# csiro-robotics/ohm

Hardware: AMD Instinct MI355X
Metric: rays/sec integrated (occupancy) (higher is better)
Workload: dtype f64

## Files before the change

### ohm_amd/csrc/batch_run.h

```cpp
#ifndef OHMHIP_BATCH_RUN_H
#define OHMHIP_BATCH_RUN_H

namespace
{
struct BatchRun
{
  ohmhip_map_t m;
  const double *d_rays;
  const float *d_intensities;
  const double *d_timestamps;
  uint32_t n_rays;
  unsigned ray_flags;
  hipStream_t s, f;
  const Event *tev;
  uint32_t ring;
  uint32_t next_info_index = 0;
  bool info_clean = false;
  uint32_t ray_blocks = 0, bin_rays_per_block = 0, bin_threads = 0, bin_blocks = 0, bin_tab_mask = 0;
  uint32_t batch_chunk_segments = 0;
  int mode = 0;
  bool stop_mode = false, occupancy_mode = false, ndt_mode = false, tsdf_mode = false;
  bool occ_inline = false;
  int ray_shift = 0;
  SecondaryLayers sec;
  int attempt = 0;
  uint32_t spec_seg_cap = 0, seg_cap = 0;
  bool speculated = false, bucket_hits = false;
  bool binned_early = false;
  BatchInfo info;
  unsigned long long *keys_a = nullptr, *keys_b = nullptr, *events = nullptr;
  const unsigned long long *sorted = nullptr;
  uint32_t event_capacity = 0, n_events = 0;
  float *direct_occ = nullptr;
  uint32_t direct_segments = 0;
  uint32_t sort_covers = 0;
  bool batch_end_marked = false;
  bool events_speculated = false;
  uint32_t spec_events = 0;

  uint32_t walkLdsHits() const { return uint32_t(m->walk_half ? WalkHalf::kLdsHits : WalkFull::kLdsHits); }

  void mark(int k) { m->tev_mask[ring] = uint8_t(m->tev_mask[ring] | (1u << k)); }

  int prepare()
  {
    m->tev_mask[ring] = 0;
    m->tev_pre_walk[ring] = 0;
    m->info_index = (m->info_index + 1u) % 3u;
    next_info_index = (m->info_index + 1u) % 3u;
    info_clean = m->info_clean;
    m->info_clean = false;
    m->parity ^= 1u;
    ray_blocks = (n_rays + 255) / 256;
    bin_rays_per_block = m->bin_rays_per_block;
    bin_threads = kBinThreads;
    while (bin_rays_per_block > 128 && n_rays / bin_rays_per_block < 2 * m->walk_workgroups)
    {
      bin_rays_per_block /= 2;
    }
    bin_threads = std::min<uint32_t>(bin_threads, bin_rays_per_block);
    bin_blocks = (n_rays + bin_rays_per_block - 1) / bin_rays_per_block;
    bin_tab_mask = std::min<uint32_t>(kLtabSize, std::max<uint32_t>(256u, 2u * bin_rays_per_block)) - 1u;
    const uint64_t expected_segments = uint64_t(double(n_rays) * m->segments_per_ray);
    batch_chunk_segments = m->chunk_segments;
    const uint32_t chunk_floor = (n_rays <= 16384u) ? std::min<uint32_t>(m->min_chunk_segments, 512u) : m->min_chunk_segments;
    while (batch_chunk_segments > chunk_floor &&
           expected_segments / batch_chunk_segments < 3ull * m->walkSlots())
    {
      batch_chunk_segments /= 2;
    }
    mode = m->config.mode;
    stop_mode = mode == OHMHIP_MODE_OCCUPANCY && (ray_flags & OHMHIP_RF_STOP_ON_FIRST_OCCUPIED) != 0;
    occupancy_mode = mode == OHMHIP_MODE_OCCUPANCY && !stop_mode;
    ndt_mode = mode == OHMHIP_MODE_NDT_OM || mode == OHMHIP_MODE_NDT_TM;
    tsdf_mode = mode == OHMHIP_MODE_TSDF;
    if (ndt_mode)
    {
      ray_flags &= (OHMHIP_RF_END_POINT_AS_FREE | OHMHIP_RF_EXCLUDE_ORIGIN | OHMHIP_RF_EXCLUDE_RAY);
    }
    if (tsdf_mode)
    {
      ray_flags = OHMHIP_RF_END_POINT_AS_FREE;
    }
    ray_shift = occupancy_mode ? 0 : kEvRayShift;
    sec.traversal = tsdf_mode ? nullptr : static_cast<float *>(m->pool.layers[OHMHIP_LID_TRAVERSAL].get());
    sec.touch_time = tsdf_mode ? nullptr : static_cast<uint32_t *>(m->pool.layers[OHMHIP_LID_TOUCH_TIME].get());
    sec.incident = tsdf_mode ? nullptr : static_cast<uint32_t *>(m->pool.layers[OHMHIP_LID_INCIDENT].get());
    sec.timestamps = d_timestamps;
    sec.time_base = m->first_ray_time;
    occ_inline = occupancy_mode && !m->pool.layers[OHMHIP_LID_MEAN] && !sec.traversal && !sec.touch_time && !sec.incident &&
                 !m->pool.layers[OHMHIP_LID_INTENSITY] && !m->pool.layers[OHMHIP_LID_HIT_MISS];

    for (int p = 0; p < 2; ++p)
    {
      OHMHIP_CHECK(m->walks_buf[p].ensure(sizeof(RayWalk) * size_t(n_rays), false, s));
      OHMHIP_CHECK(m->wg_regions[p].ensure(sizeof(WgRegion) * size_t(bin_blocks) * kLtabSize, false, s));
      OHMHIP_CHECK(m->wg_region_count[p].ensure(sizeof(uint32_t) * size_t(bin_blocks), false, s));
    }
    if (occupancy_mode)
    {
      OHMHIP_CHECK(m->hit_keys_a.ensure(sizeof(unsigned long long) * size_t(n_rays), false, s));
      OHMHIP_CHECK(m->hit_keys_b.ensure(sizeof(unsigned long long) * size_t(n_rays), false, s));
      OHMHIP_CHECK(m->interval_counts.ensure(sizeof(uint32_t) * size_t(n_rays), true, s));
      size_t sort_bytes = 0;
      OHMHIP_CHECK(rocprim::radix_sort_keys<SortConfig>(nullptr, sort_bytes, static_cast<unsigned long long *>(m->hit_keys_a.ptr),
                                            static_cast<unsigned long long *>(m->hit_keys_b.ptr), size_t(n_rays),
                                            kHitRayBits, sortEndBit(m), s));
      OHMHIP_CHECK(m->sort_temp.ensure(sort_bytes, false, s));
    }
    return OHMHIP_OK;
  }

  uint32_t *binMask() const { return occupancy_mode ? nullptr : m->pool.d_hit_mask.get(); }

  void launchBin(bool bucket, uint32_t seg_capacity, unsigned long long *hit_keys, hipStream_t stream)
  {
    const auto pow2 = [](int v) { return (v & (v - 1)) == 0; };
    const bool plain = m->mc.owner_world <= 1u && pow2(m->mc.dim[0]) && pow2(m->mc.dim[1]) && pow2(m->mc.dim[2]);
    const bool small = bin_tab_mask < kLtabSmall;
    const auto kernel = small ? (plain ? k_ray_bin<kLtabSmall, true> : k_ray_bin<kLtabSmall, false>) :
                                (plain ? k_ray_bin<kLtabSize, true> : k_ray_bin<kLtabSize, false>);
    hipExtLaunchKernelGGL(kernel, dim3(bin_blocks), dim3(bin_threads), 0, stream, nullptr, tev[1], 0, m->mc,
                          regionTable(m), batchScratch(m), static_cast<const RayWalk *>(batchWalks(m).ptr), n_rays,
                          static_cast<Segment *>(m->segments.ptr), seg_capacity, hit_keys, binMask(), ray_shift,
                          bucket ? 1 : 0, bin_rays_per_block, bin_tab_mask);
    mark(1);
    m->tev_pre_walk[ring] = 1;
    m->bin_done_event = tev[1];
  }

  uint32_t sortGrid(uint32_t per_cu) const
  {
    const uint32_t grid = per_cu * m->walk_workgroups;
    return m->sort_workgroups ? std::min(grid, m->sort_workgroups) : grid;
  }

  void launchRegionSort(uint32_t dense)
  {
    const unsigned long long *in = static_cast<const unsigned long long *>(m->hit_keys_a.ptr);
    unsigned long long *out = static_cast<unsigned long long *>(m->hit_keys_b.ptr);
    const bool need_dense = kSortSmallHits == 0 || dense > kSortSmallHits;
    if (need_dense)
    {
      hipExtLaunchKernelGGL((k_sort_region_hits<kSortRegionHits, kSortThreads>), dim3(sortGrid(2)),
                            dim3(kSortThreads), 0, s, nullptr, kSortSmallHits ? nullptr : tev[2].handle, 0, regionTable(m),
                            batchScratch(m), in, out, m->mc.region_voxels, kSortSmallHits, m->pool.d_hit_mask.get(),
                            m->d_order_counts.get());
    }
    if (kSortSmallHits)
    {
      hipExtLaunchKernelGGL((k_sort_region_hits<kSortSmallHits ? kSortSmallHits : 64u, kSortSmallThreads>),
                            dim3(sortGrid(8)), dim3(kSortSmallThreads), 0, s, nullptr, tev[2], 0,
                            regionTable(m), batchScratch(m), in, out, m->mc.region_voxels, 0u, m->pool.d_hit_mask.get(),
                            m->d_order_counts.get());
    }
    sort_covers = need_dense ? kSortRegionHits : kSortSmallHits;
    mark(2);
    m->tev_pre_walk[ring] = 2;
  }

  void launchDenseSort()
  {
    hipExtLaunchKernelGGL((k_sort_region_hits<kSortRegionHits, kSortThreads>), dim3(sortGrid(2)),
                          dim3(kSortThreads), 0, s, nullptr, tev[2], 0, regionTable(m), batchScratch(m),
                          static_cast<const unsigned long long *>(m->hit_keys_a.ptr),
                          static_cast<unsigned long long *>(m->hit_keys_b.ptr), m->mc.region_voxels, kSortSmallHits,
                          m->pool.d_hit_mask.get(), m->d_order_counts.get());
    sort_covers = kSortRegionHits;
  }

  int frontHalf()
  {
    if (m->batch_done_event[m->parity])
    {
      OHMHIP_CHECK(hipStreamWaitEvent(f, m->batch_done_event[m->parity], 0));
    }
    if (m->bin_done_event)
    {
      OHMHIP_CHECK(hipStreamWaitEvent(f, m->bin_done_event, 0));
    }
    if (attempt > 0 || !info_clean)
    {
      OHMHIP_CHECK(hipMemsetAsync(m->d_info + m->info_index, 0, sizeof(BatchInfo), f));
    }
    if (m->phase_timing)
    {
      OHMHIP_CHECK(hipEventRecord(tev[0], f));
      mark(0);
    }
    if (bin_tab_mask < kLtabSmall)
    {
      hipLaunchKernelGGL(k_ray_setup<kLtabSmall>, dim3(bin_blocks), dim3(bin_threads), 0, f, m->mc, regionTable(m),
                         batchScratch(m), d_rays, n_rays, ray_flags, static_cast<RayWalk *>(batchWalks(m).ptr),
                         bin_rays_per_block, bin_tab_mask);
    }
    else
    {
      hipLaunchKernelGGL(k_ray_setup<kLtabSize>, dim3(bin_blocks), dim3(bin_threads), 0, f, m->mc, regionTable(m),
                         batchScratch(m), d_rays, n_rays, ray_flags, static_cast<RayWalk *>(batchWalks(m).ptr),
                         bin_rays_per_block, bin_tab_mask);
    }
    hipExtLaunchKernelGGL(k_plan, dim3(1), dim3(1024), 0, f, nullptr, tev[5], 0, regionTable(m), batchScratch(m),
                          batchChunks(m), m->pool.chunk_capacity, batch_chunk_segments, m->h_info.dev,
                          m->d_info + next_info_index, batchEventCount(m), occ_inline ? walkLdsHits() : 0u);
    mark(5);
    m->info_clean = true;
    hipEvent_t plan_done = tev[5];
    if (m->spill_enabled)
    {
      OHMHIP_CHECK(queueUseStamps(m, f));
      OHMHIP_CHECK(hipEventRecord(m->ev[7], f));
      plan_done = m->ev[7];
    }
    OHMHIP_CHECK(hipStreamWaitEvent(s, plan_done, 0));
    spec_seg_cap = uint32_t(std::min<size_t>(m->segments.bytes / sizeof(Segment), 0xffffffffu));
    speculated = occupancy_mode && m->spec_bucket_ok && attempt == 0 && spec_seg_cap > 0;
    binned_early = speculated && m->early_bin && m->early_bin_event != nullptr;
    hipStream_t bin_stream = binned_early ? f : s;
    if (binned_early)
    {
      OHMHIP_CHECK(hipStreamWaitEvent(f, m->early_bin_event, 0));
    }
    if (m->phase_timing)
    {
      OHMHIP_CHECK(hipEventRecord(tev[6], bin_stream));
      mark(6);
    }
    if (speculated)
    {
      launchBin(true, spec_seg_cap, static_cast<unsigned long long *>(m->hit_keys_a.ptr), bin_stream);
      if (binned_early)
      {
        OHMHIP_CHECK(hipStreamWaitEvent(s, tev[1], 0));
        hipExtLaunchKernelGGL(k_stream_marker, dim3(1), dim3(64), 0, s, nullptr, tev[7], 0);
        m->bin_done_event = tev[7];
      }
      launchRegionSort(m->spec_max_region_hits);
    }
    OHMHIP_CHECK(hipEventSynchronize(plan_done));
    OHMHIP_CHECK(hipGetLastError());
    info = *m->h_info;
    return OHMHIP_OK;
  }

  bool exhausted() const
  {
    return (info.error & (kErrSlotsFull | kErrHashFull)) || info.n_slots > m->pool.slot_capacity ||
           info.n_chunks > m->pool.chunk_capacity;
  }

  int resolveExhaustion(bool &retry)
  {
    retry = false;
    OHMHIP_CHECK(hipStreamSynchronize(s));
    m->spec_bucket_ok = false;
    const int err = growPool(m, info.n_slots, m->pool.slot_capacity * 2u, m->slots_committed);
    if (err)
    {
      const int rollback_err = rollbackTable(m);
      if (rollback_err)
      {
        return rollback_err;
      }
      if (err == OHMHIP_ERR_CAPACITY && m->spill_enabled && !(info.error & kErrHashFull) &&
          info.n_slots > m->slots_committed)
      {
        const uint64_t allowed = poolBudget(m).regions;
        const uint64_t wanted = uint64_t(info.n_slots);
        m->batch_exceeds_limit = wanted > allowed && wanted - allowed > m->slots_committed;
        if (wanted > allowed && wanted - allowed <= m->slots_committed)
        {
          const int evict_err = evictColdRegions(m, uint32_t(wanted - allowed));
          if (evict_err == OHMHIP_OK)
          {
            retry = true;
            return OHMHIP_OK;
          }
        }
      }
      return err;
    }
    retry = true;
    return OHMHIP_OK;
  }

  int commitRegions()
  {
    m->cache_misses += info.n_slots - m->slots_committed;
    m->cache_hits += info.n_touched - std::min(info.n_touched, info.n_slots - m->slots_committed);
    if (!m->spilled.empty())
    {
      OHMHIP_CHECK(readmitSpilledSlots(m, m->slots_committed, info.n_slots));
    }
    m->slots_committed = info.n_slots;
    if (speculated && (info.n_segments > spec_seg_cap || info.max_region_hits > kSortRegionHits))
    {
      OHMHIP_CHECK(hipStreamSynchronize(s));
      if (info.n_touched)
      {
        hipLaunchKernelGGL(k_reset_cursors, dim3((info.n_touched + 255) / 256), dim3(256), 0, s, regionTable(m),
                           batchScratch(m));
      }
      speculated = false;
      binned_early = false;
    }
    return OHMHIP_OK;
  }

  int sizeBuffers()
  {
    OHMHIP_CHECK(m->segments.ensure(sizeof(Segment) * size_t(std::max<uint32_t>(info.n_segments, 1u)), false, s));
    seg_cap = uint32_t(std::min<size_t>(m->segments.bytes / sizeof(Segment), 0xffffffffu));

    uint64_t want_events =
      std::max<uint64_t>({ uint64_t(1) << 20, info.visits / 4, uint64_t(m->event_demand) * 5 / 4 });
    want_events = std::min<uint64_t>(want_events, 0xfffffff0ull - n_rays);
    if (occupancy_mode)
    {
      const uint64_t have = m->events.bytes / sizeof(unsigned long long);
      if (have >= std::max<uint64_t>(uint64_t(1) << 20, 16ull * n_rays))
      {
        want_events = std::max<uint64_t>(std::min(want_events, have), uint64_t(m->event_demand) * 5 / 4);
      }
    }
    if (m->event_limit)
    {
      want_events = std::min<uint64_t>(want_events, m->event_limit);
    }
    keys_a = keys_b = events = nullptr;
    event_capacity = 0;
    if (occupancy_mode)
    {
      OHMHIP_CHECK(m->events.ensure(sizeof(unsigned long long) * size_t(want_events), false, s));
      keys_a = static_cast<unsigned long long *>(m->hit_keys_a.ptr);
      keys_b = static_cast<unsigned long long *>(m->hit_keys_b.ptr);
      events = static_cast<unsigned long long *>(m->events.ptr);
      event_capacity = uint32_t(std::min<size_t>(m->events.bytes / sizeof(unsigned long long), 0xfffffff0u));
    }
    else
    {
      const size_t total = size_t(n_rays) + size_t(want_events);
      OHMHIP_CHECK(m->hit_keys_a.ensure(sizeof(unsigned long long) * total, false, s));
      OHMHIP_CHECK(m->hit_keys_b.ensure(sizeof(unsigned long long) * total, false, s));
      keys_a = static_cast<unsigned long long *>(m->hit_keys_a.ptr);
      keys_b = static_cast<unsigned long long *>(m->hit_keys_b.ptr);
      events = keys_a + n_rays;
      const size_t cap_a = m->hit_keys_a.bytes / sizeof(unsigned long long) - n_rays;
      const size_t cap_b = m->hit_keys_b.bytes / sizeof(unsigned long long) - n_rays;
      event_capacity = uint32_t(std::min<size_t>(std::min(cap_a, cap_b), 0xfffffff0u - n_rays));
      if (m->event_limit)
      {
        event_capacity = std::min(event_capacity, m->event_limit);
      }
    }
    return OHMHIP_OK;
  }

  int binAndOrder()
  {
    bucket_hits = occupancy_mode && info.max_region_hits <= kSortRegionHits;
    m->spec_bucket_ok = bucket_hits;
    m->spec_max_region_hits = info.max_region_hits;
    if (m->debug_flags & 4096u)
    {
      std::fprintf(stderr, "[ohmhip dbg] batch: %u rays, %u segments, %u chunks, %u regions touched, %u with samples, "
                   "densest %u samples; binned speculatively: %d\n", n_rays, info.n_segments, info.n_chunks,
                   info.n_touched, info.n_hit_regions, info.max_region_hits, int(speculated));
    }
    sorted = keys_b;
    if (speculated && info.max_region_hits > sort_covers)
    {
      launchDenseSort();
    }
    if (!speculated)
    {
      launchBin(bucket_hits, seg_cap, keys_a, s);
      if (tsdf_mode)
      {
        hipExtLaunchKernelGGL(k_tsdf_flag, dim3(ray_blocks), dim3(256), 0, s, nullptr, tev[2], 0, m->mc, regionTable(m),
                              static_cast<const RayWalk *>(batchWalks(m).ptr), d_rays, n_rays, m->pool.d_hit_mask.get());
        mark(2);
        m->tev_pre_walk[ring] = 2;
      }
      if (bucket_hits)
      {
        if (info.n_hit_regions)
        {
          launchRegionSort(info.max_region_hits);
        }
      }
      else if (occupancy_mode)
      {
        size_t temp_bytes = m->sort_temp.bytes;
        OHMHIP_CHECK(rocprim::radix_sort_keys<SortConfig>(m->sort_temp.ptr, temp_bytes, keys_a, keys_b, size_t(n_rays),
                                                          kHitRayBits, sortEndBit(info.n_slots), s));
        hipExtLaunchKernelGGL(k_hit_bounds, dim3(ray_blocks), dim3(256), 0, s, nullptr, tev[2], 0, sorted,
                              batchScratch(m), m->mc.region_voxels, m->pool.d_hit_mask.get());
        mark(2);
        m->tev_pre_walk[ring] = 2;
      }
    }
    return OHMHIP_OK;
  }

  int walk(int first_attempt = 0)
  {
    direct_occ = (occupancy_mode || mode == OHMHIP_MODE_NDT_OM) ? static_cast<float *>(m->pool.layers[OHMHIP_LID_OCCUPANCY].get()) :
                                                                  nullptr;
    direct_segments = (direct_occ || tsdf_mode) ? batch_chunk_segments : 0u;
    n_events = 0;
    if (info.n_chunks)
    {
      for (int walk_attempt = first_attempt; walk_attempt < 4; ++walk_attempt)
      {
        if (walk_attempt > 0)
        {
          OHMHIP_CHECK(hipMemsetAsync(batchEventCount(m), 0, 2 * sizeof(uint32_t), s));
        }
        WalkArgs wa;
        wa.mc = m->mc;
        wa.bs = batchScratch(m);
        wa.chunks = batchChunks(m);
        wa.segments = static_cast<const Segment *>(m->segments.ptr);
        wa.walks = static_cast<const RayWalk *>(batchWalks(m).ptr);
        wa.slot_keys = m->pool.d_slot_keys;
        wa.sorted_hits = sorted;
        wa.hit_mask = m->pool.d_hit_mask;
        wa.miss_counts = m->pool.d_miss_counts;
        wa.interval_counts = static_cast<uint32_t *>(m->interval_counts.ptr);
        wa.events = events;
        wa.event_capacity = event_capacity;
        wa.event_count = batchEventCount(m);
        wa.refill_min_idle = m->refill_min_idle;
        wa.dbg = m->debug_flags;
        wa.ray_shift = ray_shift;
        wa.defer_all = occupancy_mode ? 0 : 1;
        wa.occupancy = direct_occ;
        wa.tsdf = tsdf_mode ? static_cast<float *>(m->pool.layers[OHMHIP_LID_TSDF].get()) : nullptr;
        wa.ray_flags = ray_flags;
        const bool trace = (m->debug_flags & (16u | 64u | 128u)) != 0;
        wa.dbg_counters = trace ? m->d_dbg : nullptr;
        wa.chunk_cursor = batchEventCount(m) + 1;
        wa.n_chunks = info.n_chunks;
        wa.rewalk = (walk_attempt > 0 && (direct_occ || tsdf_mode)) ? 1 : 0;
        wa.flag_all =
          ((tsdf_mode && (m->mc.tsdf_dropoff > 0 || m->mc.tsdf_max_weight > kTsdfCountedWeightLimit)) || stop_mode) ? 1 : 0;
        wa.inline_hits = occ_inline ? 1 : 0;
        const bool traversal_pass = sec.traversal != nullptr && walk_attempt == 0;
        const bool special = (ray_flags & OHMHIP_RF_EXCLUDE_ORIGIN) != 0;
        const dim3 wgrid(std::min<uint32_t>(info.n_chunks, m->walkSlots()));
        const dim3 wblock(m->walk_half ? WalkHalf::kThreads : WalkFull::kThreads);
        const size_t wlds = walkLdsBytes(m->mc, m->chunk_segments, m->walk_half);
        hipEvent_t walk_stop = traversal_pass ? nullptr : tev[3].handle;
        if (m->walk_half)
        {
          if (special)
          {
            hipExtLaunchKernelGGL((k_region_walk<true, false, WalkHalf>), wgrid, wblock, wlds, s, nullptr, walk_stop, 0, wa);
          }
          else if (trace)
          {
            hipExtLaunchKernelGGL((k_region_walk<false, true, WalkHalf>), wgrid, wblock, wlds, s, nullptr, walk_stop, 0, wa);
          }
          else
          {
            hipExtLaunchKernelGGL((k_region_walk<false, false, WalkHalf>), wgrid, wblock, wlds, s, nullptr, walk_stop, 0, wa);
          }
        }
        else if (special)
        {
// ... 353 lines not shown
```

### ohm_amd/csrc/sample_sort_kernels.h

```cpp
#ifndef OHMHIP_SAMPLE_SORT_KERNELS_H
#define OHMHIP_SAMPLE_SORT_KERNELS_H

#include "batch_scratch.h"
#include "region_table.h"

namespace ohmhip
{
__global__ void __launch_bounds__(256)
  k_hit_bounds(const unsigned long long *__restrict__ sorted, BatchScratch bs, int region_voxels,
               uint32_t *__restrict__ hit_mask)
{
  const uint32_t n_hits = bs.info->n_hits;
  const uint32_t i = blockIdx.x * blockDim.x + threadIdx.x;
  if (i >= n_hits)
  {
    return;
  }
  const unsigned long long group = hitGroup(sorted[i]);
  if (i == 0 || hitGroup(sorted[i - 1]) != group)
  {
    const uint32_t slot = hitSlot(sorted[i]);
    const uint32_t vi = hitVoxel(sorted[i]);
    bs.voxel_first_hit[size_t(slot) * size_t(region_voxels) + vi] = i;
    atomicOr(&hit_mask[size_t(slot) * (uint32_t(region_voxels + 31) >> 5) + (vi >> 5)], 1u << (vi & 31));
  }
  const uint32_t slot = hitSlot(sorted[i]);
  if (i == 0 || hitSlot(sorted[i - 1]) != slot)
  {
    bs.hit_begin[slot] = i;
  }
  if (i + 1 == n_hits || hitSlot(sorted[i + 1]) != slot)
  {
    bs.hit_end[slot] = i + 1;
  }
}

__device__ inline uint32_t sortSlot(uint32_t i)
{
  return i + (i >> 5);
}

template <int R>
__device__ inline void bitonicFused(unsigned long long *l_keys, uint32_t g, uint32_t s_shift, uint32_t k)
{
  constexpr uint32_t kCount = 1u << R;
  const uint32_t low = g & ((1u << s_shift) - 1u);
  const uint32_t base = ((g >> s_shift) << (s_shift + R)) | low;
  const bool ascending = (base & k) == 0;
  unsigned long long v[kCount];
#pragma unroll
  for (uint32_t m = 0; m < kCount; ++m)
  {
    v[m] = l_keys[sortSlot(base | (m << s_shift))];
  }
#pragma unroll
  for (int t = 0; t < R; ++t)
  {
    const uint32_t d = 1u << (R - 1 - t);
#pragma unroll
    for (uint32_t m = 0; m < kCount; ++m)
    {
      if ((m & d) == 0)
      {
        const unsigned long long a = v[m];
        const unsigned long long c = v[m | d];
        const bool swap = (a > c) == ascending;
        v[m] = swap ? c : a;
        v[m | d] = swap ? a : c;
      }
    }
  }
#pragma unroll
  for (uint32_t m = 0; m < kCount; ++m)
  {
    l_keys[sortSlot(base | (m << s_shift))] = v[m];
  }
}

template <int kThreads>
__device__ inline void bitonicNetwork(unsigned long long *l_keys, uint32_t padded, uint32_t tid)
{
  for (uint32_t k = 2; k <= padded; k <<= 1)
  {
    uint32_t j = k >> 1;
    while (j > 0)
    {
      const uint32_t levels_left = uint32_t(32 - __clz(int(j)));
      const uint32_t r = min(3u, levels_left);
      const uint32_t s_shift = levels_left - r;
      const uint32_t group_count = padded >> r;
      for (uint32_t g = tid; g < group_count; g += kThreads)
      {
        if (r == 3)
        {
          bitonicFused<3>(l_keys, g, s_shift, k);
        }
        else if (r == 2)
        {
          bitonicFused<2>(l_keys, g, s_shift, k);
        }
        else
        {
          bitonicFused<1>(l_keys, g, s_shift, k);
        }
      }
      __syncthreads();
      j >>= r;
    }
  }
}

constexpr uint32_t kSortRegionHits = 8192;
constexpr int kSortThreads = 1024;
#ifndef OHMHIP_SORT_SMALL
#define OHMHIP_SORT_SMALL 2048
#endif
constexpr uint32_t kSortSmallHits = OHMHIP_SORT_SMALL;
constexpr int kSortSmallThreads = 256;

#ifndef OHMHIP_ORDER_SHIFT_SMALL
#define OHMHIP_ORDER_SHIFT_SMALL 5
#endif
#ifndef OHMHIP_ORDER_SHIFT_DENSE
#define OHMHIP_ORDER_SHIFT_DENSE 5
#endif
#ifndef OHMHIP_ORDER_RANK_LIMIT
#define OHMHIP_ORDER_RANK_LIMIT 32
#endif
constexpr uint32_t kOrderRankLimit = OHMHIP_ORDER_RANK_LIMIT;
static_assert(kSortRegionHits < 65536u, "bucket positions are 16-bit halves");
constexpr unsigned long long kBelowSlot = (1ull << kHitSlotShift) - 1ull;
static_assert(kSortRegionHits <= (1u << (64 - kHitSlotShift)), "a key's final position travels in its slot field");

template <uint32_t kCap, int kThreads>
__global__ void __launch_bounds__(kThreads, 8)
  k_sort_region_hits(RegionTable rt, BatchScratch bs, const unsigned long long *__restrict__ keys,
                     unsigned long long *__restrict__ sorted, int region_voxels, uint32_t min_hits,
                     uint32_t *__restrict__ hit_mask, unsigned long long *__restrict__ order_counts)
{
  constexpr uint32_t kPerLane = (kCap + uint32_t(kThreads) - 1u) / uint32_t(kThreads);
  constexpr uint32_t kWaves = uint32_t(kThreads) / 64u;
  constexpr uint32_t kOrderShift = kThreads == kSortThreads ? OHMHIP_ORDER_SHIFT_DENSE : OHMHIP_ORDER_SHIFT_SMALL;
  constexpr uint32_t kOrderWords = ((1u << kHitVoxelBits) >> kOrderShift) / 2u;
  constexpr uint32_t kScanLanes = uint32_t(kThreads) < kOrderWords ? uint32_t(kThreads) : kOrderWords;
  constexpr uint32_t kScanWords = kOrderWords / kScanLanes;
  static_assert(kThreads % 64 == 0 && kCap <= kSortRegionHits, "launch shape");
  __shared__ unsigned long long l_keys[kCap + kCap / 32];
  __shared__ uint32_t l_bucket[kOrderWords];
  __shared__ uint32_t l_wave_sum[kWaves], l_wave_sq[kWaves];
  const uint32_t mask_words = uint32_t(region_voxels + 31) >> 5;
  const uint32_t n_regions = bs.info->n_hit_regions;
  for (uint32_t list_index = blockIdx.x; list_index < n_regions; list_index += gridDim.x)
  {
  const uint32_t h = bs.sort_list[list_index];
  const uint32_t slot = rt.vals[h];
  if (slot >= rt.slot_capacity)
  {
    continue;
  }
  const uint32_t begin = bs.hit_begin[slot];
  const uint32_t n = bs.hit_end[slot] - begin;
  if (n <= min_hits || n > kCap)
  {
    continue;
  }
  uint32_t tid = threadIdx.x;
  asm volatile("" : "+v"(tid));
  const uint32_t lane = tid & 63u;
  const uint32_t wave = tid >> 6;
  for (uint32_t w = tid; w < kOrderWords; w += kThreads)
  {
    l_bucket[w] = 0;
  }
  __syncthreads();
#pragma unroll 2
  for (uint32_t i = tid; i < n; i += kThreads)
  {
    const unsigned long long key = keys[begin + i];
    l_keys[sortSlot(i)] = key;
    const uint32_t b = hitVoxel(key) >> kOrderShift;
    atomicAdd(&l_bucket[b >> 1], 1u << ((b & 1u) * 16u));
  }
  __syncthreads();
  uint32_t sum = 0, sq = 0;
#pragma unroll
  for (uint32_t w = 0; w < kScanWords; ++w)
  {
    const uint32_t word = tid < kScanLanes ? l_bucket[tid * kScanWords + w] : 0u;
    sum += (word & 0xffffu) + (word >> 16);
    sq += (word & 0xffffu) * (word & 0xffffu) + (word >> 16) * (word >> 16);
  }
  uint32_t inclusive = sum;
#pragma unroll
  for (uint32_t d = 1; d < 64u; d <<= 1)
  {
    const uint32_t up = __shfl_up(inclusive, d, 64);
    inclusive += lane >= d ? up : 0u;
    sq += __shfl_xor(sq, d, 64);
  }
  if (lane == 63u)
  {
    l_wave_sum[wave] = inclusive;
    l_wave_sq[wave] = sq;
  }
  __syncthreads();
  uint32_t position = inclusive - sum, compares = 0;
#pragma unroll
  for (uint32_t w = 0; w < kWaves; ++w)
  {
    position += w < wave ? l_wave_sum[w] : 0u;
    compares += l_wave_sq[w];
  }
  const bool ranked = kOrderRankLimit != 0 &&
                      __builtin_amdgcn_readfirstlane(compares) <= kOrderRankLimit * n;
  if (ranked)
  {
    if (tid < kScanLanes)
    {
#pragma unroll
      for (uint32_t w = 0; w < kScanWords; ++w)
      {
        const uint32_t word = l_bucket[tid * kScanWords + w];
        const uint32_t first = position;
        position += word & 0xffffu;
        l_bucket[tid * kScanWords + w] = first | (position << 16);
        position += word >> 16;
      }
    }
    __syncthreads();
#pragma unroll 2
    for (uint32_t i = tid; i < n; i += kThreads)
    {
      const unsigned long long key = keys[begin + i];
      const uint32_t b = hitVoxel(key) >> kOrderShift;
      const uint32_t half = (b & 1u) * 16u;
      const uint32_t place = (atomicAdd(&l_bucket[b >> 1], 1u << half) >> half) & 0xffffu;
      l_keys[sortSlot(place)] = key & kBelowSlot;
    }
    __syncthreads();
#pragma unroll 1
    for (uint32_t i = tid; i < n; i += kThreads)
    {
      const unsigned long long key = l_keys[sortSlot(i)];
      const uint32_t b = hitVoxel(key) >> kOrderShift;
      const uint32_t range_end = (l_bucket[b >> 1] >> ((b & 1u) * 16u)) & 0xffffu;
      const uint32_t range_begin = b ? (l_bucket[(b - 1u) >> 1] >> (((b - 1u) & 1u) * 16u)) & 0xffffu : 0u;
      uint32_t rank = 0;
#pragma unroll 4
      for (uint32_t q = range_begin; q < range_end; ++q)
      {
        const unsigned long long other = l_keys[sortSlot(q)] & kBelowSlot;
        rank += (other < key || (other == key && q < i)) ? 1u : 0u;
      }
      l_keys[sortSlot(i)] = key | ((unsigned long long)(range_begin + rank) << kHitSlotShift);
    }
    __syncthreads();
    unsigned long long own[kPerLane];
#pragma unroll
    for (uint32_t j = 0; j < kPerLane; ++j)
    {
      const uint32_t i = j * kThreads + tid;
      own[j] = i < n ? l_keys[sortSlot(i)] : 0ull;
    }
    __syncthreads();
#pragma unroll
    for (uint32_t j = 0; j < kPerLane; ++j)
    {
      if (j * kThreads + tid < n)
      {
        l_keys[sortSlot(uint32_t(own[j] >> kHitSlotShift))] =
          (own[j] & kBelowSlot) | ((unsigned long long)slot << kHitSlotShift);
      }
    }
    __syncthreads();
  }
  else
  {
    uint32_t padded = 64;
    while (padded < n)
    {
      padded <<= 1;
    }
    for (uint32_t i = n + tid; i < padded; i += kThreads)
    {
      l_keys[sortSlot(i)] = kHitInvalid;
    }
    __syncthreads();
    bitonicNetwork<kThreads>(l_keys, padded, tid);
  }
  if (threadIdx.x == 0 && order_counts)
  {
    atomicAdd(&order_counts[ranked ? 0 : 1], 1ull);
  }
  uint32_t tail_tid = threadIdx.x;
  asm volatile("" : "+v"(tail_tid));
  const uint32_t tail_lane = tail_tid & 63u;
  for (uint32_t base = 0; base < n; base += kThreads)
  {
    const uint32_t i = base + tail_tid;
    uint32_t word = 0xffffffffu, bits = 0;
    if (i < n)
    {
      const unsigned long long key = l_keys[sortSlot(i)];
      sorted[begin + i] = key;
      const uint32_t vi = hitVoxel(key);
      word = vi >> 5;
      if (i == 0 || hitGroup(l_keys[sortSlot(i - 1)]) != hitGroup(key))
      {
        bs.voxel_first_hit[size_t(slot) * size_t(region_voxels) + vi] = begin + i;
        bits = 1u << (vi & 31);
      }
    }
#pragma unroll
    for (uint32_t d = 1; d < 64u; d <<= 1)
    {
      const uint32_t up_bits = __shfl_up(bits, d, 64);
      const uint32_t up_word = __shfl_up(word, d, 64);
      bits |= (tail_lane >= d && up_word == word) ? up_bits : 0u;
    }
    const uint32_t next_word = __shfl_down(word, 1u, 64);
    if (bits && (tail_lane == 63u || next_word != word))
    {
      atomicOr(&hit_mask[size_t(slot) * mask_words + word], bits);
    }
  }
  __syncthreads();
  }
}

__global__ void k_stream_marker() {}

__global__ void __launch_bounds__(256) k_reset_cursors(RegionTable rt, BatchScratch bs)
{
  const uint32_t i = blockIdx.x * blockDim.x + threadIdx.x;
  if (i >= bs.info->n_touched)
  {
    return;
  }
  const uint32_t h = bs.touched[i];
  bs.seg_cursor[h] = 0;
  const uint32_t slot = rt.vals[h];
  if (slot < rt.slot_capacity)
  {
    bs.hit_end[slot] = bs.hit_begin[slot];
  }
}
}

#endif
```

### ohm_amd/csrc/walk_kernel.h

```cpp
#ifndef OHMHIP_WALK_KERNEL_H
#define OHMHIP_WALK_KERNEL_H

#include "batch_scratch.h"
#include "occupancy_math.h"
#include "region_table.h"
#include "walk_device.h"

namespace ohmhip
{
constexpr int kWalkThreads = 1024;
constexpr int kWalkWaves = kWalkThreads / 64;
constexpr int kQueueCap = 128;
#ifndef OHMHIP_LDS_HITS
#define OHMHIP_LDS_HITS 6144
#endif
constexpr int kLdsHits = OHMHIP_LDS_HITS;
constexpr uint32_t kIndexShift = 5;
constexpr uint32_t kIndexBuckets = (1u << kHitVoxelBits) >> kIndexShift;
constexpr int kRefillMinIdle = 20;
constexpr uint32_t kTileFlag = 0x8000u;
constexpr uint32_t kTileCountMask = 0x7fffu;
#ifndef OHMHIP_MAX_CHUNK_SEGMENTS
#define OHMHIP_MAX_CHUNK_SEGMENTS 8192
#endif
// ... 94 lines not shown
  }
}

constexpr int kFcmpOlt = 4;
constexpr int kIcmpSlt = 40;

__device__ inline int selectI(unsigned long long mask, int if_set, int if_clear)
{
  int r;
  asm("v_cndmask_b32_e64 %0, %1, %2, %3" : "=v"(r) : "v"(if_clear), "v"(if_set), "s"(mask));
  return r;
}

__device__ inline double selectD(unsigned long long mask, double if_set, double if_clear)
{
  const int lo = selectI(mask, __double2loint(if_set), __double2loint(if_clear));
  const int hi = selectI(mask, __double2hiint(if_set), __double2hiint(if_clear));
  return __hiloint2double(hi, lo);
}

__device__ inline int addMask(int value, unsigned long long mask)
{
  asm("v_addc_co_u32_e64 %0, vcc, 0, %0, %1" : "+v"(value) : "s"(mask) : "vcc");
  return value;
}

constexpr int kIcmpEq = 32;
constexpr int kIcmpUlt = 36;

__device__ inline uint32_t selectOrZero(unsigned long long mask, uint32_t if_set)
{
  uint32_t r;
  asm("v_cndmask_b32_e64 %0, 0, %1, %2" : "=v"(r) : "v"(if_set), "s"(mask));
  return r;
}

__device__ inline uint32_t umin3(uint32_t a, uint32_t b, uint32_t c)
{
  uint32_t r;
  asm("v_min3_u32 %0, %1, %2, %3" : "=v"(r) : "v"(a), "v"(b), "v"(c));
  return r;
}

__device__ inline uint32_t umed3(uint32_t a, uint32_t b, uint32_t c)
{
  uint32_t r;
  asm("v_med3_u32 %0, %1, %2, %3" : "=v"(r) : "v"(a), "v"(b), "v"(c));
  return r;
}

__device__ inline uint32_t addSat(uint32_t a, uint32_t b)
{
  uint32_t r;
  asm("v_add_u32_e64 %0, %1, %2 clamp" : "=v"(r) : "v"(a), "v"(b));
  return r;
}

__device__ inline uint32_t addSatUniform(uint32_t a, uint32_t b)
{
  uint32_t r;
  asm("v_add_u32_e64 %0, %1, %2 clamp" : "=v"(r) : "v"(a), "s"(b));
  return r;
}

__device__ inline uint32_t tileAdd(uint32_t byte_address, uint32_t value)
{
  uint32_t old;
  asm volatile("ds_add_rtn_u32 %0, %1, %2" : "=v"(old) : "v"(byte_address), "v"(value) : "memory");
  return old;
}

__device__ inline uint32_t shiftOne(uint32_t shift)
{
  uint32_t r;
  asm("v_lshlrev_b32_e64 %0, %1, 1" : "=v"(r) : "v"(shift));
  return r;
}

__device__ inline uint32_t waitTile(uint32_t old)
{
  asm volatile("s_waitcnt lgkmcnt(0)" : "+v"(old) : : "memory");
  return old;
}

struct WalkArgs
{
  MapConst mc;
  BatchScratch bs;
  const Chunk *chunks;
  const Segment *segments;
  const RayWalk *walks;
  const uint64_t *slot_keys;
  const unsigned long long *sorted_hits;
  const uint32_t *hit_mask;
  uint32_t *miss_counts;
  uint32_t *interval_counts;
  unsigned long long *events;
  uint32_t event_capacity;
  uint32_t *event_count;
  int refill_min_idle;
  unsigned dbg;
  int ray_shift;
  int defer_all;
  float *occupancy;
  unsigned ray_flags;
  unsigned long long *dbg_counters;
  float *tsdf;
  uint32_t *chunk_cursor;
  uint32_t n_chunks;
  int rewalk;
  int flag_all;
  int inline_hits;
};

constexpr uint32_t kWalkCursorWords = 24;
#ifndef OHMHIP_WALK_UNROLL
#define OHMHIP_WALK_UNROLL 2
#endif
constexpr int kWalkUnroll = OHMHIP_WALK_UNROLL;

template <int kThreadsT, int kTileVoxelsT, int kLdsHitsT, uint32_t kSegmentsT, int kQueueCapT, int kMinWavesPerEuT>
struct WalkGeometry
{
  static constexpr int kMinWavesPerEu = kMinWavesPerEuT;
  static constexpr int kThreads = kThreadsT;
  static constexpr int kWaves = kThreadsT / 64;
  static constexpr int kTileVoxels = kTileVoxelsT;
  static constexpr int kLdsHits = kLdsHitsT;
  static constexpr uint32_t kSegments = kSegmentsT;
  static constexpr int kQueueCap = kQueueCapT;
};
using WalkFull = WalkGeometry<kWalkThreads, 1 << kHitVoxelBits, kLdsHits, kMaxChunkSegments, kQueueCap, 1>;
using WalkHalf = WalkGeometry<kWalkThreads / 2, (1 << kHitVoxelBits) / 2, kLdsHits / 2, kMaxChunkSegments / 2, 96, 4>;
using LdsWord = __attribute__((address_space(3))) uint32_t;
using GlobalWord = __attribute__((address_space(1))) uint32_t;
using GlobalByte = __attribute__((address_space(1))) char;
using GlobalFloat = __attribute__((address_space(1))) float;
typedef float Float2 __attribute__((ext_vector_type(2)));
typedef uint32_t Quad __attribute__((ext_vector_type(4)));
using GlobalFloat2 = __attribute__((address_space(1))) Float2;
using LdsQuad = __attribute__((address_space(3))) Quad;

__device__ inline void addGlobal(GlobalWord *address, uint32_t value)
{
  __hip_atomic_fetch_add(address, value, __ATOMIC_RELAXED, __HIP_MEMORY_SCOPE_AGENT);
}

template <typename T>
__device__ inline T *uniformPointer(T *p)
{
  const unsigned long long v = reinterpret_cast<unsigned long long>(p);
  const uint32_t lo = __builtin_amdgcn_readfirstlane(uint32_t(v));
  const uint32_t hi = __builtin_amdgcn_readfirstlane(uint32_t(v >> 32));
  return reinterpret_cast<T *>(((unsigned long long)hi << 32) | lo);
}

__device__ inline float uniformFloat(float v)
{
  return __uint_as_float(__builtin_amdgcn_readfirstlane(__float_as_uint(v)));
}

__device__ __noinline__ void scanOrderBins(LdsWord *bins, uint32_t lane)
{
  constexpr uint32_t kQuads = kOrderBins / 256u;
  LdsQuad *mine = reinterpret_cast<LdsQuad *>(bins) + lane * kQuads;
  Quad c[kQuads];
  uint32_t total = 0;
#pragma unroll
  for (uint32_t q = 0; q < kQuads; ++q)
  {
    c[q] = mine[q];
    total += c[q].x + c[q].y + c[q].z + c[q].w;
  }
  uint32_t incl = total;
#pragma unroll
  for (int d = 1; d < 64; d <<= 1)
  {
    const uint32_t up = __shfl_up(incl, d);
    incl += (int(lane) >= d) ? up : 0u;
  }
  uint32_t run = incl - total;
#pragma unroll
  for (uint32_t q = 0; q < kQuads; ++q)
  {
    Quad e;
    e.x = run;
    e.y = e.x + c[q].x;
    e.z = e.y + c[q].y;
    e.w = e.z + c[q].z;
    run = e.w + c[q].w;
    mine[q] = e;
  }
}

template <typename G>
__device__ __noinline__ void applyFullTile(const LdsWord *tile, float *occupancy, uint32_t *g_counts, MissConst mc,
                                           unsigned long long *stamps)
{
  constexpr uint32_t kWordsPerThread = uint32_t(G::kTileVoxels) / 2u / uint32_t(G::kThreads) / 2u;
  GlobalByte *occ_bytes = (GlobalByte *)uniformPointer(occupancy);
  GlobalWord *counts = (GlobalWord *)uniformPointer(g_counts);
  stamps = uniformPointer(stamps);
  mc.miss_value = uniformFloat(mc.miss_value);
  mc.min_value = uniformFloat(mc.min_value);
  mc.sat_min = uniformFloat(mc.sat_min);
  mc.sat_max = uniformFloat(mc.sat_max);
  for (uint32_t half = 0; half < 2u; ++half)
  {
    const uint32_t first = threadIdx.x + half * kWordsPerThread * uint32_t(G::kThreads);
    uint32_t words[kWordsPerThread];
    Float2 values[kWordsPerThread];
#pragma unroll
    for (uint32_t j = 0; j < kWordsPerThread; ++j)
    {
      words[j] = tile[tileWord(first + j * uint32_t(G::kThreads))];
    }
#pragma unroll
    for (uint32_t j = 0; j < kWordsPerThread; ++j)
    {
      const uint32_t i = first + j * uint32_t(G::kThreads);
      const uint32_t sampled = ((words[j] >> 15) & 0x00010001u) * 0xffffu;
      const uint32_t kept = words[j] & sampled & (kTileCountMask | (kTileCountMask << 16));
      words[j] &= ~sampled;
      if (counts && __ballot(kept != 0u))
      {
        if (kept & 0xffffu)
        {
          addGlobal(&counts[2 * i], kept & 0xffffu);
        }
        if (kept >> 16)
        {
          addGlobal(&counts[2 * i + 1], kept >> 16);
        }
      }
      values[j] = Float2(0.0f);
      if (words[j])
      {
        values[j] = *(const GlobalFloat2 *)(occ_bytes + i * 8u);
      }
    }
#pragma unroll
    for (uint32_t j = 0; j < kWordsPerThread; ++j)
    {
      const uint32_t i = first + j * uint32_t(G::kThreads);
      if (__ballot(words[j] != 0u))
      {
        const float v0 = occMissNPlainWave(mc, values[j].x, words[j] & 0xffffu);
        if (!sameValue(v0, values[j].x))
        {
          *(GlobalFloat *)(occ_bytes + i * 8u) = v0;
        }
        const float v1 = occMissNPlainWave(mc, values[j].y, words[j] >> 16);
        if (!sameValue(v1, values[j].y))
        {
          *(GlobalFloat *)(occ_bytes + i * 8u + 4u) = v1;
        }
      }
    }
    if (stamps && threadIdx.x == 0)
    {
      stamps[half] = wall_clock64();
    }
  }
}

template <typename G>
__device__ __noinline__ void flushFullTile(const LdsWord *tile, uint32_t *g_counts, uint32_t skip_masked)
{
  constexpr uint32_t kBurst = 8;
  constexpr uint32_t kWords = uint32_t(G::kTileVoxels) / 2u / uint32_t(G::kThreads);
  static_assert(kWords % kBurst == 0u, "the tile flush reads whole bursts");
  GlobalWord *counts = (GlobalWord *)uniformPointer(g_counts);
  skip_masked = __builtin_amdgcn_readfirstlane(skip_masked);
  for (uint32_t burst = 0; burst < kWords / kBurst; ++burst)
  {
    const uint32_t first = threadIdx.x + burst * kBurst * uint32_t(G::kThreads);
    uint32_t words[kBurst];
#pragma unroll
    for (uint32_t j = 0; j < kBurst; ++j)
    {
      words[j] = tile[tileWord(first + j * uint32_t(G::kThreads))];
    }
#pragma unroll
    for (uint32_t j = 0; j < kBurst; ++j)
    {
      const uint32_t i = first + j * uint32_t(G::kThreads);
      const uint32_t masked = skip_masked ? ((words[j] >> 15) & 0x00010001u) * 0xffffu : 0u;
      const uint32_t n = words[j] & ~masked & (kTileCountMask | (kTileCountMask << 16));
      if (__ballot(n != 0u))
      {
        if (n & 0xffffu)
        {
          addGlobal(&counts[2 * i], n & 0xffffu);
        }
        if (n >> 16)
        {
          addGlobal(&counts[2 * i + 1], n >> 16);
        }
      }
    }
  }
}

template <bool kSpecial, bool kTrace, typename G = WalkFull>
__global__ void __launch_bounds__(G::kThreads, G::kMinWavesPerEu) k_region_walk(WalkArgs args)
{
  extern __shared__ __attribute__((aligned(16))) uint32_t lds[];
  const MapConst &mc = args.mc;
  const uint32_t count_words = uint32_t(mc.region_voxels + 1) >> 1;
  const uint32_t mask_words = uint32_t(mc.region_voxels + 31) >> 5;
  uint32_t *l_counts = lds;
  uint2 *l_queues = reinterpret_cast<uint2 *>(lds + ((count_words + 31u) & ~31u));
  unsigned long long *l_hits = reinterpret_cast<unsigned long long *>(l_queues + G::kWaves * G::kQueueCap);
  uint32_t *l_intervals = reinterpret_cast<uint32_t *>(l_hits + G::kLdsHits);
  uint32_t *l_cursor = l_intervals + G::kLdsHits / 2;
  uint32_t *l_idle = l_cursor + kWalkCursorWords + kLengthClasses;
  uint16_t *l_index = reinterpret_cast<uint16_t *>(l_idle + 64);
  uint16_t *l_order = l_index + kIndexBuckets + 2;
  uint32_t *l_bins = reinterpret_cast<uint32_t *>(l_queues);
  static_assert(kOrderBins <= 2u * uint32_t(G::kWaves) * uint32_t(G::kQueueCap), "the class counters alias the queues");
  static_assert(kOrderBins % 256u == 0u, "the scan gives each of 64 lanes whole uint4s");

  const int defer_all = args.defer_all;
  auto fetchNextChunk = [&](uint32_t *record, bool first = false) {
    const uint32_t next = first ? blockIdx.x : gridDim.x + atomicAdd(args.chunk_cursor, 1u);
    record[1] = next;
    if (next < args.n_chunks)
    {
      const Chunk c = args.chunks[next];
      record[2] = c.slot;
      record[3] = c.seg_begin;
      record[4] = c.seg_end;
      record[5] = c.hash_index;
      record[6] = defer_all ? 0u : args.bs.hit_begin[c.slot];
      record[7] = defer_all ? 0u : args.bs.hit_end[c.slot];
      const uint64_t key = args.slot_keys[c.slot];
      record[8] = uint32_t(key);
      record[9] = uint32_t(key >> 32);
    }
  };
  constexpr int kSegPerThread = int(G::kSegments) / G::kThreads;
  constexpr int kHitsPerThread = G::kLdsHits / uint32_t(G::kThreads);
  struct ChunkRecord
  {
    uint32_t index, slot, seg_begin, seg_end, hash_index, hb, he, key_lo, key_hi;
  };
  auto readRecord = [&](const uint32_t *record) {
    ChunkRecord r;
    r.index = __builtin_amdgcn_readfirstlane(record[1]);
    r.slot = __builtin_amdgcn_readfirstlane(record[2]);
    r.seg_begin = __builtin_amdgcn_readfirstlane(record[3]);
    r.seg_end = __builtin_amdgcn_readfirstlane(record[4]);
    r.hash_index = __builtin_amdgcn_readfirstlane(record[5]);
    r.hb = __builtin_amdgcn_readfirstlane(record[6]);
    r.he = __builtin_amdgcn_readfirstlane(record[7]);
    r.key_lo = __builtin_amdgcn_readfirstlane(record[8]);
    r.key_hi = __builtin_amdgcn_readfirstlane(record[9]);
    return r;
  };
  unsigned long long pf_hits[kHitsPerThread] = {};
  uint32_t pf_vox[kSegPerThread] = {};
  uint32_t pf_mask = 0;
  auto prefetchChunk = [&](const ChunkRecord &r) {
    const uint32_t n_hits = r.he - r.hb;
    if (!defer_all && n_hits && n_hits <= uint32_t(G::kLdsHits))
    {
#pragma unroll
      for (int j = 0; j < kHitsPerThread; ++j)
      {
        pf_hits[j] = args.sorted_hits[r.hb + min(threadIdx.x + uint32_t(j) * uint32_t(G::kThreads), n_hits - 1u)];
      }
    }
    pf_mask = args.hit_mask[size_t(r.slot) * mask_words + min(threadIdx.x, mask_words - 1u)];
    const uint32_t n = r.seg_end - r.seg_begin;
#pragma unroll
    for (int j = 0; j < kSegPerThread; ++j)
    {
      pf_vox[j] = args.segments[r.seg_begin + min(threadIdx.x + uint32_t(j) * uint32_t(G::kThreads), n - 1u)].vox;
    }
  };
  if (threadIdx.x == 0 || threadIdx.x == 64)
  {
    fetchNextChunk(l_cursor + (threadIdx.x ? kWalkCursorWords / 2 : 0), threadIdx.x == 0);
  }
  __syncthreads();
  ChunkRecord cur = readRecord(l_cursor);
  ChunkRecord next = readRecord(l_cursor + kWalkCursorWords / 2);
  if (next.index < cur.index)
  {
    const ChunkRecord swap = cur;
    cur = next;
    next = swap;
  }
  if (cur.index < args.n_chunks)
  {
    prefetchChunk(cur);
  }
  __syncthreads();
  while (cur.index < args.n_chunks)
  {
    unsigned long long clk_start = 0;
    if (kTrace)
    {
      clk_start = wall_clock64();
    }
    const uint32_t chunk_index = cur.index;
    Chunk chunk;
    chunk.slot = cur.slot;
    chunk.seg_begin = cur.seg_begin;
    chunk.seg_end = cur.seg_end;
    chunk.hash_index = cur.hash_index;
    const uint32_t hb = cur.hb;
    const uint32_t he = cur.he;
    const int region_x = int(int16_t(cur.key_lo & 0xffffu));
    const int region_y = int(int16_t(cur.key_lo >> 16));
    const int region_z = int(int16_t(cur.key_hi & 0xffffu));
    const uint32_t n_seg = chunk.seg_end - chunk.seg_begin;
    const Segment *chunk_segments = args.segments + chunk.seg_begin;

    const uint32_t n_region_hits = he - hb;
    const bool lds_resolve = !defer_all && n_region_hits <= uint32_t(G::kLdsHits);
    unsigned long long my_hits[kHitsPerThread];
#pragma unroll
    for (int j = 0; j < kHitsPerThread; ++j)
    {
      my_hits[j] = pf_hits[j];
    }
    const uint32_t *g_mask = args.hit_mask + size_t(chunk.slot) * mask_words;
    const uint32_t my_mask = pf_mask;
    uint32_t bins[kSegPerThread];
#pragma unroll
    for (int j = 0; j < kSegPerThread; ++j)
    {
      bins[j] = (kLengthClasses - 1u - min(pf_vox[j] >> kSegVoxelBits, kLengthClasses - 1u)) * kOrderCopies +
                (threadIdx.x & (kOrderCopies - 1u));
    }
    for (uint32_t b = threadIdx.x; b < kOrderBins; b += uint32_t(G::kThreads))
    {
      l_bins[b] = 0;
    }
    if (threadIdx.x == 0)
    {
      l_cursor[0] = 0;
    }
    if (threadIdx.x < 64)
    {
      l_idle[threadIdx.x] = 0;
    }
    const bool stamp = kTrace && threadIdx.x == 0;
    unsigned long long clk_p[6] = { 0, 0, 0, 0, 0, 0 };
    if (stamp)
    {
      clk_p[0] = wall_clock64();
    }
    for (uint32_t w = threadIdx.x; w < mask_words; w += uint32_t(G::kThreads))
    {
      const uint32_t mword = args.flag_all ? 0xffffffffu : ((w == threadIdx.x) ? my_mask : g_mask[w]);
      const uint32_t swizzle = tileWord(w * 16u) ^ (w * 16u);
#pragma unroll
      for (uint32_t q = 0; q < 4; ++q)
      {
        const uint32_t logical = w * 16u + q * 4u;
        if (logical + 3u < count_words)
        {
          uint32_t v[4];
#pragma unroll
          for (uint32_t r = 0; r < 4; ++r)
          {
            const uint32_t two = (mword >> ((q * 4u + (r ^ (swizzle & 3u))) * 2u)) & 3u;
            v[r] = ((two & 1u) << 15) | ((two & 2u) << 30);
          }
          *reinterpret_cast<uint4 *>(&l_counts[logical ^ (swizzle & ~3u)]) = make_uint4(v[0], v[1], v[2], v[3]);
        }
        else
        {
          for (uint32_t r = 0; r < 4; ++r)
          {
            if (logical + r < count_words)
            {
              const uint32_t two = (mword >> ((q * 4u + r) * 2u)) & 3u;
              l_counts[tileWord(logical + r)] = ((two & 1u) << 15) | ((two & 2u) << 30);
            }
          }
        }
      }
    }
    if (stamp)
    {
      clk_p[1] = wall_clock64();
    }
    __syncthreads();
    bool prefetched = false;
    if (stamp)
    {
      clk_p[2] = wall_clock64();
    }
#pragma unroll
    for (int j = 0; j < kSegPerThread; ++j)
    {
      if (threadIdx.x + uint32_t(j) * uint32_t(G::kThreads) < n_seg)
      {
        atomicAdd(&l_bins[bins[j]], 1u);
      }
    }
    if (lds_resolve && n_region_hits)
    {
#pragma unroll
      for (int j = 0; j < kHitsPerThread; ++j)
      {
        const uint32_t i = threadIdx.x + uint32_t(j) * uint32_t(G::kThreads);
        if (i < n_region_hits)
        {
          l_hits[i] = my_hits[j];
        }
        if (i < (n_region_hits + 1) / 2)
        {
          l_intervals[i] = 0;
        }
      }
    }
    __syncthreads();
    if (stamp)
    {
      clk_p[3] = wall_clock64();
    }
    if (lds_resolve && n_region_hits)
    {
#pragma unroll
      for (int j = 0; j < kHitsPerThread; ++j)
      {
        const uint32_t i = threadIdx.x + uint32_t(j) * uint32_t(G::kThreads);
        if (i < n_region_hits)
        {
          auto bucketOf = [](unsigned long long key) {
            return (uint32_t(key >> kHitRayBits) & ((1u << kHitVoxelBits) - 1u)) >> kIndexShift;
          };
          const uint32_t b = bucketOf(my_hits[j]);
          const uint32_t first = (i == 0) ? 0u : bucketOf(l_hits[i - 1]) + 1u;
          for (uint32_t k = first; k <= b; ++k)
          {
            l_index[k] = uint16_t(i);
          }
          if (i + 1 == n_region_hits)
          {
            for (uint32_t k = b + 1u; k <= kIndexBuckets; ++k)
            {
              l_index[k] = uint16_t(n_region_hits);
            }
          }
        }
      }
    }
    if (threadIdx.x < 64)
    {
      scanOrderBins((LdsWord *)l_bins, threadIdx.x);
    }
    __syncthreads();
#pragma unroll
    for (int j = 0; j < kSegPerThread; ++j)
    {
      const uint32_t i = threadIdx.x + uint32_t(j) * uint32_t(G::kThreads);
      if (i < n_seg)
      {
        l_order[atomicAdd(&l_bins[bins[j]], 1u)] = uint16_t(i);
      }
    }
    __syncthreads();
    if (stamp)
    {
      clk_p[4] = wall_clock64();
      if (chunk_index < kTraceChunks)
      {
        unsigned long long *rec = args.dbg_counters + 16 + size_t(chunk_index) * kTraceWords;
        rec[20] = clk_p[0];
        rec[21] = clk_p[1];
        rec[22] = clk_p[2];
        rec[23] = clk_p[3];
      }
    }

    const unsigned lane = laneId();
    const unsigned wave = threadIdx.x >> 6;
    uint2 *queue = l_queues + wave * G::kQueueCap;
    const int dimx = mc.dim[0];
    const int dimxy = mc.dim[0] * mc.dim[1];
    const unsigned long long slot_bits = (unsigned long long)chunk.slot << kHitSlotShift;
    const int ray_shift = args.ray_shift;
    const int refill_min_idle = args.refill_min_idle;
    const bool refill_only = kTrace && (args.dbg & 16u) != 0;
    const uint32_t fix_margin = mc.fix_margin;
    const uint32_t idle_address = uint32_t(reinterpret_cast<char *>(l_idle + lane) - reinterpret_cast<char *>(lds));

    int left = 0;
    uint32_t f0 = 0, f1 = 0, f2 = 0, d0 = 0, d1 = 0, d2 = 0;
    int sx = 0, sy = 0, sz = 0;
    uint32_t va = 0;
    uint32_t ray = 0;
    uint32_t skip = 0;
    uint32_t end_last = 0;
    uint32_t qcount = 0;
    bool exhausted = false;
    uint32_t dbg_iters = 0, dbg_active = 0, dbg_refills = 0, dbg_fm = 0, dbg_slow = 0;
    uint32_t dbg_s2 = 0, dbg_s3 = 0, dbg_sl = 0, dbg_sp = 0;
    unsigned long long clk_loop = 0;
    if (kTrace)
    {
      clk_loop = wall_clock64();
    }

    int refill_threshold = refill_min_idle;
    while (true)
    {
      const unsigned long long am = __ballot(left > 0);
      const int n_idle = 64 - __popcll(am);
      if (__builtin_expect(n_idle >= refill_threshold, 0))
      {
        if (exhausted)
        {
          break;
        }
        if (kTrace)
        {
          ++dbg_refills;
        }
        uint32_t base = 0;
        if (lane == 0)
        {
          base = atomicAdd(l_cursor, uint32_t(n_idle));
        }
        base = __builtin_amdgcn_readfirstlane(base);
        exhausted = base + uint32_t(n_idle) >= n_seg;
        refill_threshold = exhausted ? 64 : refill_threshold;
        const unsigned long long idle = ~am;
        const uint32_t mine =
          base + __builtin_amdgcn_mbcnt_hi(uint32_t(idle >> 32), __builtin_amdgcn_mbcnt_lo(uint32_t(idle), 0u));
        if (left <= 0 && mine < n_seg)
        {
          const uint4 *rec = reinterpret_cast<const uint4 *>(chunk_segments + l_order[mine]);
          const uint4 ra = rec[0];
          const uint4 rb = rec[1];
          f0 = ra.x;
          f1 = ra.y;
          f2 = ra.z;
          va = (ra.w & ((1u << kSegVoxelBits) - 1u)) << 1;
          left = int(ra.w >> kSegVoxelBits);
          d0 = rb.x & ~kSegNegative;
          d1 = rb.y & ~kSegNegative;
          d2 = rb.z & ~kSegNegative;
          sx = (rb.x & kSegNegative) ? -2 : 2;
          sy = (rb.y & kSegNegative) ? -2 * dimx : 2 * dimx;
          sz = (rb.z & kSegNegative) ? -2 * dimxy : 2 * dimxy;
          ray = rb.w & kSegRayMask;
          if (kSpecial)
          {
            skip = (rb.w & kSegSkipFirst) ? 1u : 0u;
            end_last = (rb.w & kSegEnd) ? 1u : 0u;
          }
          left = refill_only ? 0 : left;
        }
        if (!prefetched)
        {
          prefetched = true;
          if (next.index < args.n_chunks)
          {
            prefetchChunk(next);
          }
        }
      }

      uint32_t olds[kWalkUnroll];
      uint32_t visited[kWalkUnroll];
#pragma unroll
      for (int u = 0; u < kWalkUnroll; ++u)
      {
        const bool at_end = kSpecial && end_last && left == 1;
        const bool visit = kSpecial ? (left > 0 && (at_end || !skip)) : (left > 0);
        visited[u] = va;
        olds[u] = tileAdd(visit ? tileAddress(va) : idle_address, shiftOne(va << 3));
        if (kSpecial)
        {
          skip = 0;
        }
        if (kTrace)
        {
          ++dbg_iters;
          dbg_active += uint32_t(__popcll(__ballot(visit)));
        }

        int stride;
        {
          const uint32_t fmin = umin3(f0, f1, f2);
          const uint32_t fmed = umed3(f0, f1, f2);
          const uint32_t limit = min(fmed, kFixMaxDelta);
          const uint32_t lead = addSatUniform(fmin, fix_margin);
          const unsigned long long certain = __builtin_amdgcn_uicmp(lead, limit, kIcmpUlt);
          unsigned long long a0 = __builtin_amdgcn_uicmp(f0, fmin, kIcmpEq);
          unsigned long long a2 = __builtin_amdgcn_uicmp(f2, fmin, kIcmpEq);
          const unsigned long long slow = __ballot(left > 1) & ~certain;
          if (__builtin_expect(slow != 0, 0))
          {
            int axis = 1;
            if ((slow >> lane) & 1ull)
            {
              uint32_t r = ray;
              asm volatile("" : "+v"(r));
              axis = exactNextAxis(mc, args.walks[r], region_x, region_y, region_z, va >> 1);
            }
            a0 = (a0 & ~slow) | (slow & __ballot(axis == 0));
            a2 = (a2 & ~slow) | (slow & __ballot(axis == 2));
            if (kTrace)
            {
              ++dbg_slow;
              dbg_s2 += uint32_t(__popcll(slow & __ballot(left == 2)));
              dbg_s3 += uint32_t(__popcll(slow & __ballot(left == 3)));
              dbg_sl += uint32_t(__popcll(slow));
              dbg_sp += uint32_t(__popcll(slow & __ballot((d0 | d1 | d2) == 0u)));
            }
          }
          const unsigned long long a1 = ~(a0 | a2);
          f0 = addSat(f0, selectOrZero(a0, d0));
          f1 = addSat(f1, selectOrZero(a1, d1));
          f2 = addSat(f2, selectOrZero(a2, d2));
          stride = selectI(a2, sz, selectI(a0, sx, sy));
        }
        va += uint32_t(stride);
        left -= 1;
      }

      __builtin_amdgcn_sched_barrier(0);
#pragma unroll
      for (int u = 0; u < kWalkUnroll; ++u)
      {
        olds[u] = waitTile(olds[u]);
      }
#pragma unroll
      for (int u = 0; u < kWalkUnroll; ++u)
      {
        const bool flagged = __builtin_amdgcn_ubfe(olds[u], (visited[u] << 3) | 15u, 1u) != 0;
        const unsigned long long fm = __ballot(flagged);
        if (kTrace)
        {
          dbg_fm += fm ? 1u : 0u;
        }
        if (fm)
        {
          if (flagged)
          {
            const uint32_t pos =
              qcount + __builtin_amdgcn_mbcnt_hi(uint32_t(fm >> 32), __builtin_amdgcn_mbcnt_lo(uint32_t(fm), 0u));
            queue[pos] = make_uint2(visited[u] >> 1, ray);
          }
          qcount += uint32_t(__popcll(fm));
          if (qcount > uint32_t(G::kQueueCap - 64))
          {
            flushQueue(queue, qcount, lane, slot_bits, ray_shift, lds_resolve, l_hits, l_index, n_region_hits,
                       l_intervals, l_counts, args.events, args.event_capacity, args.event_count, defer_all, args.bs,
                       args.sorted_hits, args.miss_counts, args.interval_counts, mc.region_voxels);
            qcount = 0;
// ... 309 lines not shown
```

Baseline: 1.261 billion.

## Skip first-hit stores for LDS-resident regions and add fast full-tile count init

The sort kernel now writes voxel_first_hit to global memory only when a region's hit count exceeds the walk kernel's LDS hit capacity, on the premise that the walk rebuilds its index in LDS for smaller regions. Separately, the walk kernel gains a specialised tile-initialisation routine for regions that exactly fill one tile: each thread expands its mask word into swizzled count words with bit tricks instead of the generic loop. This cuts global stores and init instructions, but it relies on the walk never reading voxel_first_hit for small regions and on walkLdsHits() matching the walk's actual capacity.

```diff
diff --git a/ohm_amd/csrc/batch_run.h b/ohm_amd/csrc/batch_run.h
--- a/ohm_amd/csrc/batch_run.h
+++ b/ohm_amd/csrc/batch_run.h
@@ -145,14 +145,14 @@
       hipExtLaunchKernelGGL((k_sort_region_hits<kSortRegionHits, kSortThreads>), dim3(sortGrid(2)),
                             dim3(kSortThreads), 0, s, nullptr, kSortSmallHits ? nullptr : tev[2].handle, 0, regionTable(m),
                             batchScratch(m), in, out, m->mc.region_voxels, kSortSmallHits, m->pool.d_hit_mask.get(),
-                            m->d_order_counts.get());
+                            m->d_order_counts.get(), walkLdsHits());
     }
     if (kSortSmallHits)
     {
       hipExtLaunchKernelGGL((k_sort_region_hits<kSortSmallHits ? kSortSmallHits : 64u, kSortSmallThreads>),
                             dim3(sortGrid(8)), dim3(kSortSmallThreads), 0, s, nullptr, tev[2], 0,
                             regionTable(m), batchScratch(m), in, out, m->mc.region_voxels, 0u, m->pool.d_hit_mask.get(),
-                            m->d_order_counts.get());
+                            m->d_order_counts.get(), walkLdsHits());
     }
     sort_covers = need_dense ? kSortRegionHits : kSortSmallHits;
     mark(2);
@@ -165,7 +165,7 @@
                           dim3(kSortThreads), 0, s, nullptr, tev[2], 0, regionTable(m), batchScratch(m),
                           static_cast<const unsigned long long *>(m->hit_keys_a.ptr),
                           static_cast<unsigned long long *>(m->hit_keys_b.ptr), m->mc.region_voxels, kSortSmallHits,
-                          m->pool.d_hit_mask.get(), m->d_order_counts.get());
+                          m->pool.d_hit_mask.get(), m->d_order_counts.get(), walkLdsHits());
     sort_covers = kSortRegionHits;
   }
 
diff --git a/ohm_amd/csrc/sample_sort_kernels.h b/ohm_amd/csrc/sample_sort_kernels.h
--- a/ohm_amd/csrc/sample_sort_kernels.h
+++ b/ohm_amd/csrc/sample_sort_kernels.h
@@ -136,7 +136,8 @@
 __global__ void __launch_bounds__(kThreads, 8)
   k_sort_region_hits(RegionTable rt, BatchScratch bs, const unsigned long long *__restrict__ keys,
                      unsigned long long *__restrict__ sorted, int region_voxels, uint32_t min_hits,
-                     uint32_t *__restrict__ hit_mask, unsigned long long *__restrict__ order_counts)
+                     uint32_t *__restrict__ hit_mask, unsigned long long *__restrict__ order_counts,
+                     uint32_t walk_lds_hits)
 {
   constexpr uint32_t kPerLane = (kCap + uint32_t(kThreads) - 1u) / uint32_t(kThreads);
   constexpr uint32_t kWaves = uint32_t(kThreads) / 64u;
@@ -307,7 +308,10 @@
       word = vi >> 5;
       if (i == 0 || hitGroup(l_keys[sortSlot(i - 1)]) != hitGroup(key))
       {
-        bs.voxel_first_hit[size_t(slot) * size_t(region_voxels) + vi] = begin + i;
+        if (n > walk_lds_hits)
+        {
+          bs.voxel_first_hit[size_t(slot) * size_t(region_voxels) + vi] = begin + i;
+        }
         bits = 1u << (vi & 31);
       }
     }
diff --git a/ohm_amd/csrc/walk_kernel.h b/ohm_amd/csrc/walk_kernel.h
--- a/ohm_amd/csrc/walk_kernel.h
+++ b/ohm_amd/csrc/walk_kernel.h
@@ -420,6 +420,33 @@
   }
 }
 
+template <typename G>
+__device__ __noinline__ void initFullTile(LdsWord *tile, uint32_t mask_word, uint32_t tid)
+{
+  static_assert(uint32_t(G::kTileVoxels) == 32u * uint32_t(G::kThreads), "one mask word per thread");
+  const uint32_t w = tid;
+  const uint32_t swizzle = ((w >> 1) ^ (w >> 6)) & 31u;
+  uint32_t m = mask_word;
+  uint32_t d = (m ^ (m >> 2)) & 0x33333333u & (0u - (swizzle & 1u));
+  m ^= d ^ (d << 2);
+  d = (m ^ (m >> 4)) & 0x0f0f0f0fu & (0u - ((swizzle >> 1) & 1u));
+  m ^= d ^ (d << 4);
+  LdsQuad *groups = reinterpret_cast<LdsQuad *>(tile);
+  const uint32_t group = swizzle >> 2;
+#pragma unroll
+  for (uint32_t q = 0; q < 4; ++q)
+  {
+    Quad v;
+#pragma unroll
+    for (uint32_t r = 0; r < 4; ++r)
+    {
+      const uint32_t top = m << (30u - (q * 4u + r) * 2u);
+      v[r] = uint32_t(int32_t(top) >> 15) & 0x80008000u;
+    }
+    groups[(w * 4u + q) ^ group] = v;
+  }
+}
+
 template <bool kSpecial, bool kTrace, typename G = WalkFull>
 __global__ void __launch_bounds__(G::kThreads, G::kMinWavesPerEu) k_region_walk(WalkArgs args)
 {
@@ -571,7 +598,12 @@
     {
       clk_p[0] = wall_clock64();
     }
-    for (uint32_t w = threadIdx.x; w < mask_words; w += uint32_t(G::kThreads))
+    const bool full_init = !args.flag_all && mc.region_voxels == G::kTileVoxels;
+    if (full_init)
+    {
+      initFullTile<G>((LdsWord *)l_counts, my_mask, threadIdx.x);
+    }
+    for (uint32_t w = full_init ? mask_words : threadIdx.x; w < mask_words; w += uint32_t(G::kThreads))
     {
       const uint32_t mword = args.flag_all ? 0xffffffffu : ((w == threadIdx.x) ? my_mask : g_mask[w]);
       const uint32_t swizzle = tileWord(w * 16u) ^ (w * 16u);
```

Result: faster. 1.315 billion (median of 6 runs) (+4.3%).
